# open-speech/HTK

Hardware: AMD Instinct MI355X
Metric: herest_gmm_frame_state_loglik_per_sec (higher is better)
Workload: dtype f32 (scores: bf16x3 split operands, fp32 accumulate) + f64 (alpha / beta with fp32-transcendental log-add, accumulators); 1 GPU; HERest EM iteration (pass + accumulator all-reduce + model update), 5000 tied states x 16 mix, D=39, 1250 x 500-frame utterances per GPU (BASELINE config[2]: 10k utterances sharded 8-way); states=5000, mix=16, utts_per_gpu=1250, frames=500, chunks=1, update=HERest -m 3 -v 0.01, on the device

## Files before the change

### htk_amd/csrc/fb.hip

```cpp
#include <hip/hip_runtime.h>
#include <cstdio>
#include <cstdlib>
#include <cstring>
#include <cmath>
#include <algorithm>
#include <vector>
#include <thread>
#include <mutex>
#include <condition_variable>
#include <functional>
#include "internal.h"
#include "hipcheck.h"
#include "kernels.h"
#include "devbuf.h"

static constexpr char fbOwner[] = "fb";
typedef DevBufT<fbOwner> DevBuf;

struct PrepPool {
   std::vector<std::thread> th;
   std::mutex mu;
   std::condition_variable cvGo, cvDone;
   std::function<void(int)> job;
   int generation = 0, pending = 0, nJobs = 0;
// ... 117 lines not shown
   int nUtt = 0;
   int debug = 0;
   int forceGeneral = 0;
   int noStatePath = 0;
   int noLrPath = 0;
   int topoVersion = 0;
   std::vector<unsigned char> uttFlags;
   UttClasses cls;
   size_t gamTotal = 0, betaWTotal = 0, alphaWTotal = 0;
   int totalFrames = 0, nCellsMax = 1, QMax = 1, TMax = 1, blockDim = 64;
   long long frameStates = 0;
   const float *dX = nullptr;
   DevBuf d_arena;
   DevBuf d_qLo, d_qHi, d_aLo, d_aHi, d_outp, d_beta, d_gam, d_alpha, d_pr;
   DevBuf d_betaW;
   DevBuf d_tmE, d_tmMaxP;
   DevBuf d_outpU;
   DevBuf d_alphaW, d_qBeam, d_aBeam, d_trPart, d_hits, d_hitCtl;
   DevBuf d_sink;
   DevBuf d_stCnt, d_stBucket;
   DevBuf d_laneRec;
   bool mixStateLast = false;
   bool mixDeferred = false;
   FbArgs *faMix = nullptr;
   const int *qBeamLast = nullptr;
   DevBuf d_transOff, d_trOccOff, d_counter;
   DevBuf d_rec, d_recSorted, d_recCtl;
   int recCapForce = 0;
   PrepPool *pool = nullptr; std::vector<PrepChunk> *chunks = nullptr;
   void *h_arena = nullptr; size_t h_arenaCap = 0;
   void *h_res = nullptr; size_t h_resCap = 0;
   hipEvent_t evRes = nullptr; bool resPending = false;
   bool f16Pass = false;
   hipEvent_t ev[6] = {}, evK[2] = {}, evCopy = nullptr;
   hipStream_t resStream = nullptr;
   bool timed = false, copyPending = false, scored = false;
   int evMode = 0, evModeLast = 0;
   ResLayout res() const { return {(size_t)nUtt}; }
};

static bool compat_revisit(const htkamd_model *m) { return (m->compat & HTKAMD_COMPAT_STREAM_REVISIT) && m->NSt > 1 && m->NSt != 3 && !m->tiedMix; }

extern "C" int htkamd_fb_create(htkamd_model *m, htkamd_fb **out)
{
   if (!m || !out) { htkamd_set_error("fb_create: NULL argument"); return HTKAMD_EINVAL; }
   if (m->fullc) { htkamd_set_error("fb_create: forward-backward on FULLC models is not supported yet (its mixture statistics are diagonal)"); return HTKAMD_EMODEL; }
   if (m->maxM > 4096) { htkamd_set_error("fb_create: %d mixture components per state not supported", m->maxM); return HTKAMD_EMODEL; }
   htkamd_fb *fb = new htkamd_fb();
   fb->m = m;
   auto fail = [&](const char *what, hipError_t e) { htkamd_set_error("fb_create: %s: %s", what, hipGetErrorString(e)); htkamd_fb_destroy(fb); return HTKAMD_EHIP; };
   hipError_t e;
   for (hipEvent_t *v : {&fb->ev[0], &fb->ev[1], &fb->ev[2], &fb->ev[3], &fb->ev[4], &fb->ev[5], &fb->evK[0], &fb->evK[1]})
      if ((e = hipEventCreate(v)) != hipSuccess) return fail("hipEventCreate", e);
   if ((e = hipEventCreateWithFlags(&fb->evCopy, hipEventDisableTiming)) != hipSuccess) return fail("hipEventCreate", e);
   if ((e = hipStreamCreateWithFlags(&fb->resStream, hipStreamNonBlocking)) != hipSuccess) return fail("hipStreamCreate", e);
   int rc;
   if ((rc = fb->d_counter.reserve(64)) || (rc = fb->d_transOff.reserve(sizeof(int) * (m->nT + 1))) || (rc = fb->d_trOccOff.reserve(sizeof(int) * (m->nT + 1)))) { htkamd_fb_destroy(fb); return rc; }
   if ((e = hipMemcpy(fb->d_transOff.p, m->h_transOff, sizeof(int) * (m->nT + 1), hipMemcpyHostToDevice)) != hipSuccess ||
       (e = hipMemcpy(fb->d_trOccOff.p, m->h_trOccOff, sizeof(int) * (m->nT + 1), hipMemcpyHostToDevice)) != hipSuccess) return fail("hipMemcpy", e);
   *out = fb;
   return HTKAMD_OK;
}

extern "C" void htkamd_fb_destroy(htkamd_fb *fb)
{
   if (!fb) return;
// ... 445 lines not shown

static const int clsW[4] = {1, 2, 4, 8};

static int fb_reserve_lr(htkamd_fb *fb, const htkamd_fb_config *cfg, FbArgs &fa, bool fastLadd, hipStream_t s)
{
   const htkamd_model *m = fb->m;
   int rc;
   size_t rows = 0;
   for (int W : clsW) rows += (size_t)fb->cls.of(FB_LEFT_TO_RIGHT, W).n * htkamd_stats_lr_chunks(fb->TMax) * W;
   const size_t nfr = fb->totalFrames ? fb->totalFrames : 1;
   if ((rc = fb->d_laneRec.reserve(sizeof(LaneRec) * (fb->slotState.size() + 1))) || (rc = fb->d_sink.reserve(256))) return rc;
   fa.laneRec = (LaneRec *)fb->d_laneRec.p; fa.sink = (double *)fb->d_sink.p;
   if ((rc = fb->d_alphaW.reserve(sizeof(double) * (fb->alphaWTotal + 64))) || (rc = fb->d_qBeam.reserve(sizeof(int) * (nfr + 2))) ||
       (rc = fb->d_aBeam.reserve(sizeof(int) * (nfr + 2))) || (rc = fb->d_trPart.reserve(sizeof(double) * htkamd_stats_lr_row_doubles() * (rows + 256))) ||
       (rc = fb->d_hits.reserve(sizeof(MixHit) * (rows * htkamd_stats_lr_region_cap() + 64))) || (rc = fb->d_hitCtl.reserve(sizeof(int) * (rows + 1))))
      return rc;
   fa.alphaW = (double *)fb->d_alphaW.p; fa.qBeam = (int *)fb->d_qBeam.p; fa.aBeam = (int *)fb->d_aBeam.p; fa.trPart = (double *)fb->d_trPart.p;
   fa.hits = (MixHit *)fb->d_hits.p; fa.hitCtl = (int *)fb->d_hitCtl.p; fa.nHitRegions = (int)rows; fa.hitRegionCap = htkamd_stats_lr_region_cap();
   fa.hitSlots = (m->NSt > 1 || m->tiedMix) ? 1 : 0;
   fa.qBeamNP = fb->qBeamNP.dev;
   if (htkamd_beta_lr_is_lean(fa, fastLadd)) fa.qBeam = const_cast<int *>(fb->qBeamNP.dev);
   fb->qBeamLast = fa.qBeam;
   fb->mixStateLast = false;
   fa.fastMath = fastLadd ? 1 : 0;
   if (fb->recCapForce == 0 && !fa.hitSlots && m->maxM <= 16 && (m->D == 39 || m->D == 26 || m->D == 13) &&
       (cfg->uFlags & (HTKAMD_UPMEANS | HTKAMD_UPVARS | HTKAMD_UPMIXES))) {
      size_t cap = 64;
      while (cap < 65536 && cap * (size_t)m->S < (size_t)16 * fb->totalFrames) cap <<= 1;
      while (cap > 64 && cap * (size_t)m->S * sizeof(HitS) > ((size_t)1 << 30)) cap >>= 1;
      { const char *e = getenv("HTKAMD_ST_CAP"); if (e && atoi(e) > 0) cap = (size_t)atoi(e); }
      if ((rc = fb->d_stCnt.reserve(sizeof(int) * (3 * (size_t)m->S + 4))) || (rc = fb->d_stBucket.reserve(sizeof(HitS) * cap * (size_t)m->S))) return rc;
      fb->mixStateLast = true;
      fa.stCnt = (int *)fb->d_stCnt.p; fa.nTiedStates = m->S; fa.stBucket = (HitS *)fb->d_stBucket.p; fa.stCap = (int)cap;
      HIPCHECK(hipMemsetAsync(fa.stCnt, 0, sizeof(int) * (3 * (size_t)m->S + 4), s));
   }
   return HTKAMD_OK;
}

struct FamilyKernels { int family; int (*beta)(const FbArgs &, int, bool, hipStream_t); int (*alpha)(const FbArgs &, int, bool, hipStream_t); };
static const FamilyKernels familyKernels[] = {{FB_LANE_PER_MODEL, htkamd_launch_beta_w, htkamd_launch_alpha_w},
                                              {FB_LANE_PER_STATE, htkamd_launch_beta_s, htkamd_launch_alpha_s},
                                              {FB_LEFT_TO_RIGHT, htkamd_launch_beta_lr, htkamd_launch_alpha_lr}};

static int fb_recursions(htkamd_fb *fb, const FbArgs &fa, const LdsSizes &lds, bool fastLadd, bool noEv, hipStream_t s)
{
   int rc;
   for (int pass = 0; pass < 2; pass++) {
      FbArgs fc = fa;
      const UttClasses::Range g = fb->cls.general();
      fc.uttList = fb->uttList.dev + g.first; fc.nList = g.n;
      if (g.n > 0 && (rc = pass == 0 ? htkamd_launch_beta(fc, fb->blockDim, lds.beta, s) : htkamd_launch_alpha(fc, fb->blockDim, lds.alpha, s))) return rc;
      for (const FamilyKernels &k : familyKernels)
         for (int c = 3; c >= 0; c--) {
            const UttClasses::Range r = fb->cls.of(k.family, clsW[c]);
            fc.uttList = fb->uttList.dev + r.first; fc.nList = r.n;
            if ((rc = (pass == 0 ? k.beta : k.alpha)(fc, clsW[c], fastLadd, s))) return rc;
         }
      if (!noEv) HIPCHECK(hipEventRecord(fb->ev[2 + pass], s));
   }
   return HTKAMD_OK;
}

static int fb_stats_lr(htkamd_fb *fb, const FbArgs &fa, bool fastLadd, bool noEv, hipStream_t s)
{
   int rc;
   FbArgs fc = fa;
   size_t rowOff = 0;
   for (int c = 3; c >= 0; c--) {
      const UttClasses::Range r = fb->cls.of(FB_LEFT_TO_RIGHT, clsW[c]);
      fc.uttList = fb->uttList.dev + r.first; fc.nList = r.n;
      fc.trPart = fa.trPart ? fa.trPart + rowOff * htkamd_stats_lr_row_doubles() : nullptr;
      fc.hits = fa.hits ? fa.hits + rowOff * htkamd_stats_lr_region_cap() : nullptr; fc.hitCtl = fa.hitCtl ? fa.hitCtl + rowOff : nullptr;
      rowOff += (size_t)fc.nList * htkamd_stats_lr_chunks(fb->TMax) * clsW[c];
      if ((rc = htkamd_launch_stats_lr(fc, clsW[c], fastLadd, s))) return rc;
   }
   if (!noEv) HIPCHECK(hipEventRecord(fb->ev[4], s));
   return HTKAMD_OK;
}

static int fb_mix_stats(htkamd_fb *fb, const htkamd_fb_config *cfg, FbArgs &fa, bool defer, hipStream_t s)
{
   const htkamd_model *m = fb->m;
   const int nLr = fb->cls.nLr();
   int rc;
   if (!(cfg->uFlags & (HTKAMD_UPMEANS | HTKAMD_UPVARS | HTKAMD_UPMIXES))) return HTKAMD_OK;
   if ((cfg->uFlags & (HTKAMD_UPMEANS | HTKAMD_UPVARS)) && fb->recCapForce >= 0) {
      const size_t cap = fb->recCapForce > 0 ? (size_t)fb->recCapForce : std::min<size_t>((size_t)16 * fb->totalFrames + 4096, (size_t)1 << 30);
      if ((rc = fb->d_rec.reserve(sizeof(MixRec) * cap)) || (rc = fb->d_recSorted.reserve(sizeof(MixRec) * cap)) ||
          (rc = fb->d_recCtl.reserve(sizeof(int) * (3 * ((size_t)m->G + 1) + 1 + (size_t)m->G / 2048 + 2))))
         return rc;
      fa.rec = (MixRec *)fb->d_rec.p; fa.recSorted = (MixRec *)fb->d_recSorted.p; fa.recCap = (int)cap; fa.G = m->G; fa.recCtl = (int *)fb->d_recCtl.p;
   }
   if (m->tiedMix || m->NSt > 1) {
      fa.stateCompOff = m->d_stateCompOff; fa.rec = nullptr;
      if (fb->nUtt > nLr && (rc = m->tiedMix ? htkamd_launch_mixstats_tm(fa, s) : htkamd_launch_mixstats_ms(fa, s))) return rc;
      if (nLr > 0 && (rc = htkamd_launch_mixhits_streams(fa, m->tiedMix != 0, s))) return rc;
      return HTKAMD_OK;
   }
   const bool dense = fb->nUtt > nLr && fa.gamTotal > 0, listed = nLr > 0;
   if ((rc = htkamd_launch_mixstats(fa, s, dense, listed, defer))) return rc;
   if (defer && listed && !dense && htkamd_mixstate_applies(fa)) {
      if (!fb->faMix) fb->faMix = new FbArgs();
      *fb->faMix = fa;
      fb->mixDeferred = true;
   }
   return HTKAMD_OK;
}

static int fb_execute_impl(htkamd_fb *fb, const htkamd_fb_config *cfg, htkamd_accs *accs, void *stream, bool defer)
{
   if (!fb || !cfg || !accs) { htkamd_set_error("fb_execute: NULL argument"); return HTKAMD_EINVAL; }
   fb->mixDeferred = false;
   if (accs->m != fb->m) { htkamd_set_error("fb_execute: accumulators belong to a different model"); return HTKAMD_EINVAL; }
   if (fb->nUtt == 0) return HTKAMD_OK;
   const htkamd_model *m = fb->m;
   hipStream_t s = (hipStream_t)stream;
   if (fb->topoVersion != m->topoVersion) {
      htkamd_set_error("fb_execute: the model's minimum durations changed since htkamd_fb_prepare (a re-estimated transition reached or left zero): prepare the batch again");
      return HTKAMD_EINVAL;
   }
   const ScoreArgs sa = fb_score_args(fb, cfg);
   if (cfg->scoreMode & ~(HTKAMD_SCORE_MFMA | HTKAMD_SCORE_FASTLADD | HTKAMD_SCORE_BF16 | HTKAMD_SCORE_F16 | HTKAMD_SCORE_SOUTP | HTKAMD_SCORE_DIAGC)) { htkamd_set_error("fb_execute: unknown score mode %d", cfg->scoreMode); return HTKAMD_EINVAL; }
   const bool fastLadd = (cfg->scoreMode & HTKAMD_SCORE_FASTLADD) != 0;
   FbArgs fa = fb_args(fb, cfg, accs);
   const LdsSizes lds = fb_lds_sizes(fa);

   int rc;
   if (fb->copyPending) HIPCHECK(hipStreamWaitEvent(s, fb->evCopy, 0));
   const bool noEv = fb->evMode == 1;
   HIPCHECK(hipEventRecord(fb->ev[0], s));
   if (m->tiedMix) {
      fa.tmE = (float *)fb->d_tmE.p; fa.tmMaxP = (float *)fb->d_tmMaxP.p; fa.tmPoolOff = m->d_tmPoolOff; fa.tmPool = m->tmPool; fa.totalFrames = fb->totalFrames;
      fa.tmTasks = fb->tasks.dev; fa.tmNTasks = (int)fb->tasks.size(); fa.tmSlotState = sa.slotState; fa.tmOut = sa.out;
      fa.compWeight = m->d_compWeight; fa.var = m->d_var;
      if ((rc = htkamd_launch_tm_score(fa, s))) return rc;
      fb->scored = false;
   } else {
      if ((rc = htkamd_launch_score(cfg->scoreMode, m, sa, s, fb->evK[0], fb->evK[1]))) return rc;
      fb->scored = sa.nTasks > 0;
   }
   if (m->NSt > 1) {
      if ((rc = htkamd_launch_combine_streams(fa, s))) return rc;
      if (m->maxM > 1) fa.stateCompOff = m->d_msCompOff;
   } else if (m->tiedMix) fa.stateCompOff = m->d_msCompOff;
   if (!noEv) HIPCHECK(hipEventRecord(fb->ev[1], s));
   if (fb->cls.nGeneral() > 0 && lds.alpha > 160 * 1024) { htkamd_set_error("fb_execute: %zu bytes of LDS needed (max model size %zu states)", lds.alpha, (size_t)m->maxN); return HTKAMD_EMODEL; }
   if ((rc = fb->d_betaW.reserve(sizeof(double) * (fb->betaWTotal + 8 * 512)))) return rc;
   fa.betaW = (double *)fb->d_betaW.p;
   if (fb->cls.nLr() > 0 && (rc = fb_reserve_lr(fb, cfg, fa, fastLadd, s))) return rc;
   if ((rc = fb_recursions(fb, fa, lds, fastLadd, noEv, s)) || (rc = fb_stats_lr(fb, fa, fastLadd, noEv, s)) || (rc = fb_mix_stats(fb, cfg, fa, defer, s))) return rc;
   HIPCHECK(hipEventRecord(fb->ev[5], s));
   fb->timed = true; fb->evModeLast = noEv ? 1 : 0;
   return HTKAMD_OK;
}

extern "C" int htkamd_fb_execute(htkamd_fb *fb, const htkamd_fb_config *cfg, htkamd_accs *accs, void *stream)
{
   return fb_execute_impl(fb, cfg, accs, stream, false);
}

extern "C" int htkamd_fb_execute_begin(htkamd_fb *fb, const htkamd_fb_config *cfg, htkamd_accs *accs, void *stream, int *deferred)
{
   if (deferred) *deferred = 0;
   const int rc = fb_execute_impl(fb, cfg, accs, stream, true);
   if (rc == HTKAMD_OK && deferred && fb && fb->nUtt > 0) *deferred = fb->mixDeferred ? 1 : 0;
   return rc;
}

extern "C" int htkamd_fb_execute_mix(htkamd_fb *fb, int state0, int state1, void *stream)
{
   if (!fb) { htkamd_set_error("fb_execute_mix: NULL"); return HTKAMD_EINVAL; }
   if (fb->nUtt == 0 || !fb->mixDeferred) return HTKAMD_OK;
   const int rc = htkamd_launch_mixstate_range(*fb->faMix, state0, state1, (hipStream_t)stream);
   if (rc) return rc;
   HIPCHECK(hipEventRecord(fb->ev[5], (hipStream_t)stream));
   return HTKAMD_OK;
}


static int res_staging(htkamd_fb *fb, size_t bytes)
{
   if (bytes > fb->h_resCap) {
      if (fb->h_res) (void)hipHostFree(fb->h_res);
      fb->h_res = nullptr; fb->h_resCap = 0;
      HIPCHECK(hipHostMalloc(&fb->h_res, bytes + bytes / 4, hipHostMallocDefault));
      fb->h_resCap = bytes + bytes / 4;
   }
   return HTKAMD_OK;
}

extern "C" int htkamd_fb_results_begin(htkamd_fb *fb, void *stream)
{
   if (!fb) { htkamd_set_error("fb_results_begin: NULL"); return HTKAMD_EINVAL; }
   if (fb->nUtt == 0) return HTKAMD_OK;
   hipStream_t s = (hipStream_t)stream;
   const size_t bytes = fb->res().bytes();
   int rc = res_staging(fb, bytes);
   if (rc) return rc;
   if (!fb->evRes) HIPCHECK(hipEventCreateWithFlags(&fb->evRes, hipEventDisableTiming));
   HIPCHECK(hipMemcpyAsync(fb->h_res, fb->d_pr.p, bytes, hipMemcpyDeviceToHost, s));
   HIPCHECK(hipEventRecord(fb->evRes, s));
   fb->resPending = true;
   return HTKAMD_OK;
}

extern "C" int htkamd_fb_results(htkamd_fb *fb, double *pr, int *status, void *stream)
{
   if (!fb) { htkamd_set_error("fb_results: NULL"); return HTKAMD_EINVAL; }
   hipStream_t s = (hipStream_t)stream;
   if (fb->nUtt == 0) return HTKAMD_OK;
   const size_t bytes = fb->res().bytes();
   if (fb->resPending) {
      fb->resPending = false;
      HIPCHECK(hipEventSynchronize(fb->evRes));
   } else {
      int rc = res_staging(fb, bytes);
      if (rc) return rc;
      hipStream_t cs = fb->timed ? fb->resStream : s;
      if (fb->timed) HIPCHECK(hipEventSynchronize(fb->ev[5]));
      HIPCHECK(hipMemcpyAsync(fb->h_res, fb->d_pr.p, bytes, hipMemcpyDeviceToHost, cs));
      HIPCHECK(hipStreamSynchronize(cs));
   }
   if (pr) memcpy(pr, fb->h_res, sizeof(double) * (size_t)fb->nUtt);
   if (status) memcpy(status, (const char *)fb->h_res + fb->res().status(), sizeof(int) * (size_t)fb->nUtt);
   if (fb->f16Pass) {
      int flag;
      memcpy(&flag, (const char *)fb->h_res + fb->res().flag(), sizeof(int));
      if (flag) {
         htkamd_set_error("fb_results: the fp16 scoring path met %s%s%s outside its range: nothing of this pass can be used (accumulators included) -- repeat it with HTKAMD_SCORE_BF16",
                          (flag & HTKAMD_F16_EMODEL) ? "a model coefficient" : "", (flag & HTKAMD_F16_EMODEL) && (flag & HTKAMD_F16_EFEAT) ? " and " : "", (flag & HTKAMD_F16_EFEAT) ? "a feature value" : "");
         return HTKAMD_ERANGE;
      }
   }
// ... 151 lines not shown
```

### htk_amd/csrc/fb_lr_lean.inc

```

template <int W>
__global__ __launch_bounds__(64 * W) void k_beta_np(FbArgs a)
{
   constexpr int L = 64 * W, LP = L + 2 * SPAD;
   __shared__ double xz[2][LP];
   __shared__ double prSlot;
   const int gl = threadIdx.x;
   const int li = blockIdx.x;
   if (li >= a.nList) return;
   const int u = a.uttList[li];
   const UttDesc ud = a.utt[u];
   if (ud.status != HTKAMD_UTT_OK) {
      if (gl == 0) { a.status[u] = ud.status; a.pr[u] = LZERO; }
      return;
   }
   const int T = ud.T, Q = ud.Q, nS = ud.nSlots;
   const bool valid = gl < nS;
   LrRegs s;
   load_lr(s, a, ud, gl, valid);
   store_lane_rec(a, ud, gl, valid, s);
   for (int i = gl; i < LP; i += L) { xz[0][i] = LZERO; xz[1][i] = LZERO; }
   if (gl == 0) prSlot = LZERO;
   __syncthreads();
   const int q = s.q;
   const double dSelf = (double)s.aSelf;
   const double cN = s.last ? (double)s.aExit + (double)s.aEntryNext : (double)s.aNext;
   const double dEntry = (double)s.aEntry;
   cint_lr *wB = (cint_lr *)(a.qBeamNP + ud.frame0 - 1);
   const float *row = a.outp + ud.outp0 + (size_t)(valid ? gl : 0) * T;
   double *pB = a.betaW + ud.betaW0 + gl;

   int w = wB[T];
   int lo = w & 0xffff, hi = w >> 16;
   bool in = q >= lo && q <= hi;
   constexpr int BK = 8;
   const int bT = (T - 1) / BK;
   float Rc[BK], Rn[BK];
   auto load8 = [&](float *R, const int b) {
      const f4s lo4 = *(const f4s *)(row + BK * b), hi4 = *(const f4s *)(row + BK * b + 4);
#pragma unroll
      for (int k = 0; k < 4; k++) { R[k] = lo4[k]; R[4 + k] = hi4[k]; }
// ... 469 lines not shown
         for (int o = 32; o > 0; o >>= 1) v += __shfl_xor(v, o);
         rowv[k] = v;
      }
      if (lane == 0) {
#pragma unroll
         for (int k = 0; k < 11; k++) part[k] = wantTrans ? rowv[k] : 0.0;
         part[TR_ROW - 1] = wantTrans ? (double)t0m : -1.0;
      }
   }
}

__device__ __forceinline__ double dpp_from_next(const double v, const double edge)
{
   const long long b = __double_as_longlong(v), e = __double_as_longlong(edge);
   const int lo = __builtin_amdgcn_update_dpp((int)e, (int)b, 0x130, 0xf, 0xf, false);
   const int hi = __builtin_amdgcn_update_dpp((int)(e >> 32), (int)(b >> 32), 0x130, 0xf, 0xf, false);
   return __longlong_as_double(((long long)hi << 32) | (unsigned int)lo);
}
__device__ __forceinline__ double dpp_from_prev(const double v, const double edge)
{
   const long long b = __double_as_longlong(v), e = __double_as_longlong(edge);
   const int lo = __builtin_amdgcn_update_dpp((int)e, (int)b, 0x138, 0xf, 0xf, false);
   const int hi = __builtin_amdgcn_update_dpp((int)(e >> 32), (int)(b >> 32), 0x138, 0xf, 0xf, false);
   return __longlong_as_double(((long long)hi << 32) | (unsigned int)lo);
}
typedef double d2s __attribute__((ext_vector_type(2), aligned(8)));

#define LEAN2_EU 1
__global__ __launch_bounds__(64, LEAN2_EU) void k_beta_np2(FbArgs a)
{
   constexpr int L = 128;
   const int lane = threadIdx.x, g0 = 2 * lane, g1 = g0 + 1;
   const int li = blockIdx.x;
   if (li >= a.nList) return;
   const int u = a.uttList[li];
   const UttDesc ud = a.utt[u];
   if (ud.status != HTKAMD_UTT_OK) {
      if (lane == 0) { a.status[u] = ud.status; a.pr[u] = LZERO; }
      return;
   }
   const int T = ud.T, Q = ud.Q, nS = ud.nSlots;
   const bool v0 = g0 < nS, v1 = g1 < nS;
   LrRegs s0, s1;
   load_lr(s0, a, ud, g0, v0); load_lr(s1, a, ud, g1, v1);
   store_lane_rec(a, ud, g0, v0, s0); store_lane_rec(a, ud, g1, v1, s1);
   const int q0 = s0.q, q1 = s1.q;
   const double dSelf0 = (double)s0.aSelf, dSelf1 = (double)s1.aSelf;
   const double cN0 = s0.last ? (double)s0.aExit + (double)s0.aEntryNext : (double)s0.aNext;
   const double cN1 = s1.last ? (double)s1.aExit + (double)s1.aEntryNext : (double)s1.aNext;
   cint_lr *wB = (cint_lr *)(a.qBeamNP + ud.frame0 - 1);
   const float *row0 = a.outp + ud.outp0 + (size_t)(v0 ? g0 : 0) * T, *row1 = a.outp + ud.outp0 + (size_t)(v1 ? g1 : 0) * T;
   double *pB = a.betaW + ud.betaW0 + g0;

   int w = wB[T];
   int lo = w & 0xffff, hi = w >> 16;
   bool in0 = q0 >= lo && q0 <= hi, in1 = q1 >= lo && q1 <= hi;
   constexpr int BK = 8;
   const int bT = (T - 1) / BK;
   float Rc0[BK], Rc1[BK], Rn0[BK], Rn1[BK];
   auto load8 = [&](float *R, const float *row, const int b) {
      const f4s lo4 = *(const f4s *)(row + BK * b), hi4 = *(const f4s *)(row + BK * b + 4);
#pragma unroll
      for (int k = 0; k < 4; k++) { R[k] = lo4[k]; R[4 + k] = hi4[k]; }
   };
   auto pick = [](const float *R, int k) { float v = R[0];
#pragma unroll
// ... 279 lines not shown
```

### htk_amd/csrc/gmm_bf16.hip

```cpp
#include <hip/hip_runtime.h>
#include <hip/hip_ext.h>
#include "internal.h"
#include "hipcheck.h"
#include "kernels.h"

typedef float f4 __attribute__((ext_vector_type(4)));
typedef float f4u __attribute__((ext_vector_type(4), aligned(4)));
typedef __bf16 bf8 __attribute__((ext_vector_type(8)));
typedef unsigned int u4 __attribute__((ext_vector_type(4)));
typedef const __attribute__((address_space(4))) int cint;

#define EXP2(x) __builtin_amdgcn_exp2f(x)
#define LOG2(x) __builtin_amdgcn_logf(x)
#define B16_COL_TILES 2

__device__ __forceinline__ float rows_max_b(float v)
{
   auto a = __builtin_amdgcn_permlane16_swap(__float_as_uint(v), __float_as_uint(v), false, false);
   v = fmaxf(__uint_as_float(a[0]), __uint_as_float(a[1]));
   auto b = __builtin_amdgcn_permlane32_swap(__float_as_uint(v), __float_as_uint(v), false, false);
   return fmaxf(__uint_as_float(b[0]), __uint_as_float(b[1]));
}
__device__ __forceinline__ float rows_sum_b(float v)
{
// ... 431 lines not shown
               if (3 * ks + 1 < 18) lse_slice(3 * ks + 1);
               Cc = __builtin_amdgcn_mfma_f32_32x32x16_bf16(wa[ks][0], zb[ks][1], Cc, 0, 0, 0);
               Cc = __builtin_amdgcn_mfma_f32_32x32x16_bf16(wa[ks][1], zb[ks][0], Cc, 0, 0, 0);
               if (3 * ks + 2 < 18) lse_slice(3 * ks + 2);
               Cx = __builtin_amdgcn_mfma_f32_32x32x16_bf16(wa[ks][0], zb[ks][0], Cx, 0, 0, 0);
            }
            for (int sl = 3 * KS; sl < 18; sl++) lse_slice(sl);
            asm volatile("" : "+v"(resP));
            resQ = resP; oQ = oPrev; haveQ = prevAct;
#pragma unroll
            for (int b = 0; b < 4; b++) {
               const f4 ci = __builtin_bit_cast(f4, wbuf[buf][KS * 192 + kh * 4 + b]);
#pragma unroll
               for (int r = 0; r < 4; r++) yP[4 * b + r] = (Cx[4 * b + r] + Cc[4 * b + r]) + ci[r];
            }
         }
         prevAct = actJ; oPrev += oStep;
         asm volatile("s_waitcnt vmcnt(0)" ::: "memory");
         __syncthreads();
         buf ^= 1;
      }
      if (haveQ) { if (fw + fcol < tk.nFrames) *oQ = resQ; }
      if (prevAct) {
         const float res = lse_full();
         if (fw + fcol < tk.nFrames && 2 * (nPairs - 1) + kh < tk.nSlots) *oPrev = res;
      }
   }
}

int htkamd_launch_score_bf16(const htkamd_model *m, const ScoreArgs &a, hipStream_t stream, hipEvent_t evStart, hipEvent_t evStop)
{
   if (a.nTasks <= 0) return HTKAMD_OK;
   { const int rc = htkamd_model_table_current(m, HTKAMD_SCORE_BF16, stream); if (rc) return rc; }
   if (a.qCounters == a.taskCounter + 8) HIPCHECK(hipMemsetAsync(a.taskCounter, 0, 16 * sizeof(int), stream));
   else {
      HIPCHECK(hipMemsetAsync(a.taskCounter, 0, sizeof(int), stream));
      if (a.qCounters) HIPCHECK(hipMemsetAsync(a.qCounters, 0, 8 * sizeof(int), stream));
   }
   if (m->f16Wide && (size_t)m->nTiles * ((size_t)3 * m->bf16NC * 64 * 16 + 64 * 16) >= ((size_t)1 << 32)) {
      htkamd_set_error("score_bf16: a table of %d tiles is beyond the kernel's 32-bit staging offsets", m->nTiles); return HTKAMD_EMODEL;
   }
   if (m->f16Wide) {
      dim3 block(256);
#define W_LAUNCH(KS_) do { const int b_ = a.nTasks < 256 * b16w_eu(KS_) ? a.nTasks : 256 * b16w_eu(KS_); \
                           hipExtLaunchKernelGGL((k_score_bf16w<KS_>), dim3(b_), block, 0, stream, evStart, evStop, 0, a); } while (0)
      if (m->bf16Dense) {
         W_LAUNCH(5); HIPCHECK(hipGetLastError());
         return HTKAMD_OK;
      }
      switch (m->bf16NC) {
      case 3: W_LAUNCH(6); break;
      case 2: W_LAUNCH(4); break;
      case 1: W_LAUNCH(2); break;
      default: htkamd_set_error("score_bf16: no kernel for %d K-chunks", m->bf16NC); return HTKAMD_EMODEL;
      }
#undef W_LAUNCH
      HIPCHECK(hipGetLastError());
      return HTKAMD_OK;
   }
   const int parts = B16_TASK_FRAMES / (16 * B16_COL_TILES * B16_WPB);
   int blocks = a.nTasks * parts;
   if (blocks > 256 * ((B16_COL_TILES > 2 ? 8 : 12) / B16_WPB)) blocks = 256 * ((B16_COL_TILES > 2 ? 8 : 12) / B16_WPB);
   dim3 grid(blocks), block(64 * B16_WPB);
   switch (m->bf16NC) {
   case 3: hipExtLaunchKernelGGL((k_score_bf16<3>), grid, block, 0, stream, evStart, evStop, 0, a); break;
   case 2: hipExtLaunchKernelGGL((k_score_bf16<2>), grid, block, 0, stream, evStart, evStop, 0, a); break;
   case 1: hipExtLaunchKernelGGL((k_score_bf16<1>), grid, block, 0, stream, evStart, evStop, 0, a); break;
// ... 156 lines not shown
```

### htk_amd/csrc/kernels.h

```cpp
#ifndef HTKAMD_KERNELS_H
#define HTKAMD_KERNELS_H
#include <hip/hip_runtime.h>
#include <vector>
#include "internal.h"

#define SCORE_TILE_FRAMES 128
#define B16_TASK_FRAMES 128
#define SCORE_TASK_SLOTS  16
#define SCORE_TASK_SLOTS_WIDE 64
#define SCORE_TASK_SLOTS_EXACT 8

struct ScoreTask {
   int frame0;
   int nFrames;
   int slot0;
   int nSlots;
   int outSlot0;
   int ldo;
   size_t outBase;
};

struct ScoreArgs {
   const ScoreTask *tasks = nullptr;
   int nTasks = 0;
   const float *X = nullptr;
   const int *slotState = nullptr;
   float *out = nullptr;
   const int *stateCompOff = nullptr, *compGauss = nullptr;
   const float *compLogWt = nullptr, *gparam = nullptr;
   int PS = 0, D = 0;
   double minLogExp = 0.0;
   const double *laddTab = nullptr;
   int *taskCounter = nullptr;
   const float *mfmaTab = nullptr;
   const int *stateTileOff = nullptr;
   const void *bf16Tab = nullptr;
   const void *f16Tab = nullptr;
   const int *f16Ctl = nullptr;
   int *rangeFlag = nullptr;
   const float *var = nullptr;
   int NSt = 1;
   const float *streamWt = nullptr;
   const int *qStart = nullptr;
   int *qCounters = nullptr;
   const int *slotRange = nullptr;
};

static inline ScoreArgs htkamd_score_args(const htkamd_model *m)
{
   ScoreArgs a;
   a.stateCompOff = m->d_stateCompOff; a.compGauss = m->d_compGauss; a.compLogWt = m->d_compLogWt;
   a.gparam = m->d_gparam; a.PS = m->PS; a.D = m->D; a.minLogExp = m->minLogExp; a.laddTab = m->d_laddTab;
   a.mfmaTab = m->d_mfmaTab; a.stateTileOff = m->d_stateTileOff; a.bf16Tab = m->d_bf16Tab; a.var = m->d_var;
   a.NSt = m->NSt; a.streamWt = m->d_streamWt;
   return a;
}

static inline int htkamd_tile_count(int T, int nSlots, int FR, int SL) { return ((T + FR - 1) / FR) * ((nSlots + SL - 1) / SL); }
static inline void htkamd_tile_tasks(ScoreTask *tk, int frame0, int T, int slot0, int nSlots, size_t outBase, int ldo, int FR, int SL)
{
   for (int t0 = 0; t0 < T; t0 += FR)
      for (int k0 = 0; k0 < nSlots; k0 += SL, tk++) {
         tk->frame0 = frame0 + t0; tk->nFrames = (T - t0 < FR) ? T - t0 : FR;
         tk->slot0 = slot0 + k0; tk->nSlots = (nSlots - k0 < SL) ? nSlots - k0 : SL;
         tk->outSlot0 = k0; tk->ldo = ldo; tk->outBase = outBase + (size_t)t0;
      }
}
static inline void htkamd_tile_tasks(std::vector<ScoreTask> &v, int frame0, int T, int slot0, int nSlots, size_t outBase, int ldo, int FR, int SL)
{
   if (T <= 0 || nSlots <= 0) return;
   const size_t n = v.size();
   v.resize(n + (size_t)htkamd_tile_count(T, nSlots, FR, SL));
   htkamd_tile_tasks(v.data() + n, frame0, T, slot0, nSlots, outBase, ldo, FR, SL);
}

int htkamd_launch_score_exact(const htkamd_model *m, const ScoreArgs &a, hipStream_t stream, hipEvent_t evStart = nullptr, hipEvent_t evStop = nullptr, bool soutp = false, bool diagc = false);
int htkamd_launch_score_full(const htkamd_model *m, const ScoreArgs &a, hipStream_t stream, hipEvent_t evStart, hipEvent_t evStop, bool soutp, bool diagc);
int htkamd_launch_score_mfma(const htkamd_model *m, const ScoreArgs &a, hipStream_t stream, hipEvent_t evStart = nullptr, hipEvent_t evStop = nullptr);
// ... 70 lines not shown
   htkamd_accs_layout lay;
   double pruneInit, pruneInc, pruneLim, minLogExp;
   float minFrwdP;
   int uFlags;
   size_t gamTotal;
   const size_t *gamOffByUtt;
   const int *gamChunkUtt;
   MixRec *rec, *recSorted;
   int recCap, G;
   int *recCtl;
   int NSt;
   const float *outpU;
   int compatRevisit;
   const int *nextSame;
   const int *dimStream;
   float *tmE;
   float *tmMaxP;
   const int *tmPoolOff;
   int tmPool, totalFrames;
   const ScoreTask *tmTasks; int tmNTasks; const int *tmSlotState; float *tmOut;
   const float *compWeight, *var;
   int tmCombine;
   const float *streamWt;
   MixHit *hits;
   int hitSlots;
   int *hitCtl;
   int nHitRegions, hitRegionCap;
   LaneRec *laneRec;
   const int *qBeamNP;
   int stBase;
   int *stCnt; int nTiedStates; HitS *stBucket; int stCap;
   int fastMath;
   double *sink;
};

int htkamd_launch_beta(const FbArgs &a, int blockDim, size_t lds, hipStream_t s);
int htkamd_launch_alpha(const FbArgs &a, int blockDim, size_t lds, hipStream_t s);
int htkamd_launch_mixstats(const FbArgs &a, hipStream_t s, bool dense, bool listed, bool deferState = false);
bool htkamd_mixstate_applies(const FbArgs &a);
int htkamd_launch_mixstate_range(const FbArgs &a, int st0, int st1, hipStream_t s);
int htkamd_launch_combine_streams(const FbArgs &a, hipStream_t s);
int htkamd_launch_mixstats_ms(const FbArgs &a, hipStream_t s);
int htkamd_launch_tm_score(const FbArgs &a, hipStream_t s);
int htkamd_launch_mixstats_tm(const FbArgs &a, hipStream_t s);
int htkamd_launch_mixhits_streams(const FbArgs &a, bool tied, hipStream_t s);
int htkamd_tm_score_block(const htkamd_model *m, const ScoreArgs &sa, int nRows, float tmBeam, hipStream_t s);
int htkamd_launch_beta_s(const FbArgs &a, int W, bool fast, hipStream_t s);
int htkamd_launch_alpha_s(const FbArgs &a, int W, bool fast, hipStream_t s);
int htkamd_launch_beta_w(const FbArgs &a, int W, bool fast, hipStream_t s);
int htkamd_launch_beta_lr(const FbArgs &a, int W, bool fast, hipStream_t s);
bool htkamd_beta_lr_is_lean(const FbArgs &a, bool fast);
int htkamd_launch_alpha_lr(const FbArgs &a, int W, bool fast, hipStream_t s);
int htkamd_launch_stats_lr(const FbArgs &a, int W, bool fast, hipStream_t s);
int htkamd_stats_lr_chunks(int TMax);
size_t htkamd_stats_lr_row_doubles(void);
int htkamd_stats_lr_region_cap(void);
int htkamd_launch_alpha_w(const FbArgs &a, int W, bool fast, hipStream_t s);

#endif
```

### htk_amd/csrc/update.hip

```cpp
#include <hip/hip_runtime.h>
#include <cstdlib>
#include <cstring>
#include <cmath>
#include "internal.h"
#include "hipcheck.h"

struct UpdArgs {
   int D, S, C, G, nT, H, PS, maxM;
   const int *stateCompOff, *compGauss, *transN, *transOff, *trOccOff, *hmmTrans, *hmmStateOff, *hmmState;
   float *mean, *var, *gconst, *compWeight, *transP;
   float *ivar, *gparam, *compLogWt;
   const unsigned char *rawLogWt;
   const double *acc;
   htkamd_accs_layout lay;
   int minEgs, uFlags, singleProcess, rowNormalise, hasVarFloor;
   float minVar, mixWeightFloor;
   double logTpi;
   const float *varFloor;
   unsigned char *qualT, *qualS, *qualG, *anyS, *anyG;
   unsigned char *flooredG;
   int *stats;
   int *blkStats;
   float *logVar;
   int tied;
// ... 482 lines not shown
   const int idx = blockIdx.x * blockDim.x + threadIdx.x;
   if (idx >= nTiles * 16) return;
   const int t = idx >> 4, col = idx & 15;
   int lo = 0, hi = a.S - 1;
   while (lo < hi) { const int mid = (lo + hi + 1) >> 1; if (a.stateTileOff[mid] <= t) lo = mid; else hi = mid - 1; }
   const int s = lo, c0 = a.stateCompOff[s], c1 = a.stateCompOff[s + 1];
   const int c = c0 + 16 * (t - a.stateTileOff[s]) + col;
   const int NS = a.NS, D = a.D;
   float *T = a.tab + (size_t)t * (NS + 8) * 64;
   float *ciRow = T + (size_t)(NS + (col & 3)) * 64 + (col >> 2) * 16, *endRow = ciRow + 4 * 64;
   const bool live = c < c1 && (c1 - c0 == 1 || a.compLogWt[c] > (float)LMINMIX);
   if (!live) {
      for (int j = 0; j < 16; j++) { ciRow[j] = 0.0f; endRow[j] = -1.0e30f; }
      for (int st = 0; st < NS; st++) for (int kq = 0; kq < 4; kq++) T[(size_t)st * 64 + kq * 16 + col] = 0.0f;
      return;
   }
   const int g = a.compGauss[c];
   const float *mu = a.mean + (size_t)g * D, *iv = a.ivar + (size_t)g * D;
   double q = 0.0;
   for (int i = 0; i < D; i++) q += (double)mu[i] * mu[i] * iv[i];
   const double L2E = 1.4426950408889634;
   const float ci = (float)(-0.25 * q * L2E);
   const float ce = (float)(((c1 - c0 == 1 ? 0.0 : (double)a.compLogWt[c]) - 0.5 * (double)a.gconst[g] - 0.25 * q) * L2E);
   for (int j = 0; j < 16; j++) { ciRow[j] = ci; endRow[j] = ce; }
   for (int st = 0; st < NS; st++)
      for (int kq = 0; kq < 4; kq++) {
         const int dim = 2 * st + (kq >> 1);
         float v = 0.0f;
         if (dim < D) v = (kq & 1) ? (float)((double)mu[dim] * iv[dim] * L2E) : (float)(-0.5 * (double)iv[dim] * L2E);
         T[(size_t)st * 64 + kq * 16 + col] = v;
      }
}

__global__ void k_upd_export(const int *stats, int *dst, const int *blkStats, int nBlk)
{
   int c0 = 0, c1 = 0, c2 = 0;
   for (int i = threadIdx.x; i < nBlk; i += 64) { c0 += blkStats[3 * i]; c1 += blkStats[3 * i + 1]; c2 += blkStats[3 * i + 2]; }
#pragma unroll
   for (int o = 32; o > 0; o >>= 1) { c0 += __shfl_xor(c0, o); c1 += __shfl_xor(c1, o); c2 += __shfl_xor(c2, o); }
   if (threadIdx.x < 16) dst[threadIdx.x] = stats[threadIdx.x] + (threadIdx.x == 0 ? c0 : threadIdx.x == 1 ? c1 : threadIdx.x == 5 ? c2 : 0);
}

int htkamd_model_refresh_mfma_device(htkamd_model *m, void *stream)
{
   hipStream_t s = (hipStream_t)stream;
   if (!m->d_mfmaTab) return HTKAMD_OK;
   MfmaTabArgs t;
   t.D = m->D; t.NS = m->mfmaNS; t.S = m->S; t.stateCompOff = m->d_stateCompOff; t.stateTileOff = m->d_stateTileOff; t.compGauss = m->d_compGauss;
   t.mean = m->d_mean; t.ivar = m->d_ivar; t.gconst = m->d_gconst; t.compLogWt = m->d_compLogWt; t.tab = m->d_mfmaTab;
   const int n = m->nTiles * 16;
   hipLaunchKernelGGL(k_upd_mfma, dim3((n + 255) / 256), dim3(256), 0, s, t, m->nTiles);
   HIPCHECK(hipGetLastError());
   return HTKAMD_OK;
}

extern "C" int htkamd_model_update_device_begin(htkamd_model *m, htkamd_accs *accs, const htkamd_update_config *cfg, void *stream)
{
   if (!m || !accs || !cfg) { htkamd_set_error("model_update_device: NULL argument"); return HTKAMD_EINVAL; }
   if (accs->m != m) { htkamd_set_error("model_update_device: accumulators belong to a different model"); return HTKAMD_EINVAL; }
   if (cfg->uFlags & HTKAMD_UPMAP) { htkamd_set_error("model_update_device: MAP re-estimation (HTKAMD_UPMAP) is done by htkamd_model_update"); return HTKAMD_EMODEL; }
   hipStream_t s = (hipStream_t)stream;
   int rc;
   if ((rc = htkamd_model_device_tables(m))) return rc;
   const size_t nFlag = (size_t)m->nT + 2 * (size_t)m->S + 3 * (size_t)m->G;
   const bool tied = m->h_meanLeader != nullptr;
   const size_t nTiedInts = tied ? 2 * (size_t)m->G + (size_t)m->H : 0;
   const size_t nLog = tied ? 0 : (((size_t)m->G * m->D + 3) & ~(size_t)3);
   const size_t headBytes = (((nFlag + 63) & ~(size_t)63) + 16 * sizeof(int) + sizeof(float) * (size_t)m->D + sizeof(int) * nTiedInts + 255) & ~(size_t)255;
// ... 51 lines not shown
         hipLaunchKernelGGL(k_upd_trans, dim3((m->nT + B - 1) / B), dim3(B), 0, s, a);
         hipLaunchKernelGGL(k_upd_state, dim3((m->S + B - 1) / B), dim3(B), 0, s, a);
      }
   }
   if (m->tiedMix) HIPCHECK(hipMemsetAsync(a.qualG, 1, (size_t)m->G, s));
   bool fusedG = false;
   {
      const size_t nEl = (size_t)m->G * m->D;
      const size_t ldsFused = sizeof(float) * (size_t)UPD_GPB * (m->D + m->PS) + sizeof(int) * UPD_GPB;
      if (nEl >= ((size_t)1 << 31)) { htkamd_set_error("model_update_device: %zu mean / variance elements (the element kernel indexes with 32 bits)", nEl); return HTKAMD_EMODEL; }
      if (tied) {
         hipLaunchKernelGGL(k_upd_first, dim3((m->H + B - 1) / B), dim3(B), 0, s, a);
         hipLaunchKernelGGL(k_upd_gauss_elem_tied, dim3((unsigned)((nEl + 255) / 256)), dim3(256), 0, s, a);
      } else if (!m->tiedMix && ldsFused <= 60 * 1024 && (m->PS & 3) == 0 && m->D <= 64) {
         const dim3 gr((unsigned)((m->G + UPD_GPB - 1) / UPD_GPB));
         switch ((UPD_GPB * m->D + 1023) / 1024) {
         case 1: hipLaunchKernelGGL(k_upd_gauss_fused<1>, gr, dim3(256), ldsFused, s, a); break;
         case 2: hipLaunchKernelGGL(k_upd_gauss_fused<2>, gr, dim3(256), ldsFused, s, a); break;
         case 3: hipLaunchKernelGGL(k_upd_gauss_fused<3>, gr, dim3(256), ldsFused, s, a); break;
         default: hipLaunchKernelGGL(k_upd_gauss_fused<4>, gr, dim3(256), ldsFused, s, a); break;
         }
         fusedG = true;
      } else
         hipLaunchKernelGGL(k_upd_gauss_elem, dim3((unsigned)((nEl + 1023) / 1024)), dim3(256), 0, s, a);
   }
   if (!fusedG) {
      UpdArgs ag = a;
      if (sizeof(float) * (size_t)B * m->D > 48 * 1024) ag.logVar = nullptr;
      hipLaunchKernelGGL(k_upd_gconst, dim3((m->G + B - 1) / B), dim3(B), ag.logVar ? sizeof(float) * (size_t)B * m->D : 0, s, ag);
   }
   HIPCHECK(hipGetLastError());
   if ((rc = htkamd_model_params_changed(m, s, 1))) return rc;
   const size_t nTp = (size_t)m->h_transOff[m->nT];
   if (!m->h_updPin) HIPCHECK(hipHostMalloc(&m->h_updPin, sizeof(float) * (nTp + 16), hipHostMallocDefault));
   if (!m->evUpd) { hipEvent_t e; HIPCHECK(hipEventCreateWithFlags(&e, hipEventDisableTiming)); m->evUpd = (void *)e; }
   hipLaunchKernelGGL(k_upd_export, dim3(1), dim3(64), 0, s, a.stats, (int *)(m->d_transP + nTp), a.blkStats, fusedG ? (int)((m->G + UPD_GPB - 1) / UPD_GPB) : 0);
   HIPCHECK(hipMemcpyAsync(m->h_updPin, m->d_transP, sizeof(float) * (nTp + 16), hipMemcpyDeviceToHost, s));
   HIPCHECK(hipEventRecord((hipEvent_t)m->evUpd, s));
   free(scanPosHost);
   m->updPending = 1;
   return HTKAMD_OK;
}

extern "C" int htkamd_model_update_device_end(htkamd_model *m, htkamd_update_stats *stats)
{
   if (!m || !m->updPending) { htkamd_set_error("model_update_device_end: no update in flight"); return HTKAMD_EINVAL; }
   m->updPending = 0;
   HIPCHECK(hipEventSynchronize((hipEvent_t)m->evUpd));
   const size_t nTp = (size_t)m->h_transOff[m->nT];
   int hst[16];
   memcpy(m->h_transP, m->h_updPin, sizeof(float) * nTp);
   memcpy(hst, (const float *)m->h_updPin + nTp, sizeof(hst));
   htkamd_model_refresh_topology(m);
   if (stats) {
      stats->nFloorVar = hst[0]; stats->nFloorVarMix = hst[1]; stats->nSkippedHmm = hst[2];
      stats->nNoTransOut = hst[3]; stats->nNoMixUse = hst[4]; stats->nNoVarUse = hst[5]; stats->nWeightAboveOne = hst[6];
   }
   if (hst[6] > 0) { htkamd_set_error("model_update_device: %d mixture weights above 1.001 (HERest: HError 2393)", hst[6]); return HTKAMD_EMODEL; }
   return HTKAMD_OK;
}

extern "C" int htkamd_model_update_device(htkamd_model *m, htkamd_accs *accs, const htkamd_update_config *cfg, htkamd_update_stats *stats, void *stream)
{
   const int rc = htkamd_model_update_device_begin(m, accs, cfg, stream);
   return rc ? rc : htkamd_model_update_device_end(m, stats);
}
```

Baseline: 29.49 billion frame-state log-lik/s.

## Fold counter memsets into beta kernel and write results straight to mapped host memory

The per-state counter and score task-counter memsets are now done by the first left-to-right lean beta kernel, which zeroes those words itself. The next scoring call then skips its own memset when it knows the counters are already clean. The result and update-export device-to-host memcpys are replaced by small kernels that write directly into mapped, coherent pinned host buffers, and the ev[0] record is skipped when events are off. The aim is fewer API calls and stream operations per iteration. The cost is cross-call state that tracks whether the counters are clean, plus slower zero-copy PCIe stores from kernels.

```diff
diff --git a/htk_amd/csrc/fb.hip b/htk_amd/csrc/fb.hip
--- a/htk_amd/csrc/fb.hip
+++ b/htk_amd/csrc/fb.hip
@@ -173,6 +173,7 @@
    void *h_res = nullptr; size_t h_resCap = 0;
    hipEvent_t evRes = nullptr; bool resPending = false;
    bool f16Pass = false;
+   bool scoreCntClean = false;
    hipEvent_t ev[6] = {}, evK[2] = {}, evCopy = nullptr;
    hipStream_t resStream = nullptr;
    bool timed = false, copyPending = false, scored = false;
@@ -684,8 +685,10 @@
       if ((rc = fb->d_stCnt.reserve(sizeof(int) * (3 * (size_t)m->S + 4))) || (rc = fb->d_stBucket.reserve(sizeof(HitS) * cap * (size_t)m->S))) return rc;
       fb->mixStateLast = true;
       fa.stCnt = (int *)fb->d_stCnt.p; fa.nTiedStates = m->S; fa.stBucket = (HitS *)fb->d_stBucket.p; fa.stCap = (int)cap;
-      HIPCHECK(hipMemsetAsync(fa.stCnt, 0, sizeof(int) * (3 * (size_t)m->S + 4), s));
-   }
+      if (htkamd_beta_lr_is_lean(fa, fastLadd)) { fa.zeroW[0] = fa.stCnt; fa.nZeroW[0] = 3 * m->S + 4; }
+      else HIPCHECK(hipMemsetAsync(fa.stCnt, 0, sizeof(int) * (3 * (size_t)m->S + 4), s));
+   }
+   if (htkamd_beta_lr_is_lean(fa, fastLadd)) { fa.zeroW[1] = (int *)fb->d_counter.p; fa.nZeroW[1] = 16; }
    return HTKAMD_OK;
 }
 
@@ -697,8 +700,10 @@
 static int fb_recursions(htkamd_fb *fb, const FbArgs &fa, const LdsSizes &lds, bool fastLadd, bool noEv, hipStream_t s)
 {
    int rc;
+   bool zeroed = false;
    for (int pass = 0; pass < 2; pass++) {
       FbArgs fc = fa;
+      fc.zeroW[0] = fc.zeroW[1] = nullptr;
       const UttClasses::Range g = fb->cls.general();
       fc.uttList = fb->uttList.dev + g.first; fc.nList = g.n;
       if (g.n > 0 && (rc = pass == 0 ? htkamd_launch_beta(fc, fb->blockDim, lds.beta, s) : htkamd_launch_alpha(fc, fb->blockDim, lds.alpha, s))) return rc;
@@ -706,7 +711,10 @@
          for (int c = 3; c >= 0; c--) {
             const UttClasses::Range r = fb->cls.of(k.family, clsW[c]);
             fc.uttList = fb->uttList.dev + r.first; fc.nList = r.n;
+            const bool zeroHere = pass == 0 && k.family == FB_LEFT_TO_RIGHT && r.n > 0 && !zeroed && (fa.zeroW[0] || fa.zeroW[1]);
+            if (zeroHere) { fc.zeroW[0] = fa.zeroW[0]; fc.zeroW[1] = fa.zeroW[1]; }
             if ((rc = (pass == 0 ? k.beta : k.alpha)(fc, clsW[c], fastLadd, s))) return rc;
+            if (zeroHere) { zeroed = true; fc.zeroW[0] = fc.zeroW[1] = nullptr; if (fa.zeroW[1]) fb->scoreCntClean = true; }
          }
       if (!noEv) HIPCHECK(hipEventRecord(fb->ev[2 + pass], s));
    }
@@ -771,7 +779,9 @@
       htkamd_set_error("fb_execute: the model's minimum durations changed since htkamd_fb_prepare (a re-estimated transition reached or left zero): prepare the batch again");
       return HTKAMD_EINVAL;
    }
-   const ScoreArgs sa = fb_score_args(fb, cfg);
+   ScoreArgs sa = fb_score_args(fb, cfg);
+   sa.countersZero = fb->scoreCntClean && sa.taskCounter == (int *)fb->d_counter.p;
+   fb->scoreCntClean = false;
    if (cfg->scoreMode & ~(HTKAMD_SCORE_MFMA | HTKAMD_SCORE_FASTLADD | HTKAMD_SCORE_BF16 | HTKAMD_SCORE_F16 | HTKAMD_SCORE_SOUTP | HTKAMD_SCORE_DIAGC)) { htkamd_set_error("fb_execute: unknown score mode %d", cfg->scoreMode); return HTKAMD_EINVAL; }
    const bool fastLadd = (cfg->scoreMode & HTKAMD_SCORE_FASTLADD) != 0;
    FbArgs fa = fb_args(fb, cfg, accs);
@@ -780,7 +790,7 @@
    int rc;
    if (fb->copyPending) HIPCHECK(hipStreamWaitEvent(s, fb->evCopy, 0));
    const bool noEv = fb->evMode == 1;
-   HIPCHECK(hipEventRecord(fb->ev[0], s));
+   if (!noEv) HIPCHECK(hipEventRecord(fb->ev[0], s));
    if (m->tiedMix) {
       fa.tmE = (float *)fb->d_tmE.p; fa.tmMaxP = (float *)fb->d_tmMaxP.p; fa.tmPoolOff = m->d_tmPoolOff; fa.tmPool = m->tmPool; fa.totalFrames = fb->totalFrames;
       fa.tmTasks = fb->tasks.dev; fa.tmNTasks = (int)fb->tasks.size(); fa.tmSlotState = sa.slotState; fa.tmOut = sa.out;
@@ -830,12 +840,17 @@
 }
 
 
+__global__ __launch_bounds__(256) void k_fb_results_out(const int *__restrict__ src, int *__restrict__ dst, int nWords)
+{
+   for (int i = blockIdx.x * blockDim.x + threadIdx.x; i < nWords; i += gridDim.x * blockDim.x) dst[i] = src[i];
+}
+
 static int res_staging(htkamd_fb *fb, size_t bytes)
 {
    if (bytes > fb->h_resCap) {
       if (fb->h_res) (void)hipHostFree(fb->h_res);
       fb->h_res = nullptr; fb->h_resCap = 0;
-      HIPCHECK(hipHostMalloc(&fb->h_res, bytes + bytes / 4, hipHostMallocDefault));
+      HIPCHECK(hipHostMalloc(&fb->h_res, bytes + bytes / 4, hipHostMallocMapped | hipHostMallocCoherent));
       fb->h_resCap = bytes + bytes / 4;
    }
    return HTKAMD_OK;
@@ -850,7 +865,11 @@
    int rc = res_staging(fb, bytes);
    if (rc) return rc;
    if (!fb->evRes) HIPCHECK(hipEventCreateWithFlags(&fb->evRes, hipEventDisableTiming));
-   HIPCHECK(hipMemcpyAsync(fb->h_res, fb->d_pr.p, bytes, hipMemcpyDeviceToHost, s));
+   void *dRes = nullptr;
+   HIPCHECK(hipHostGetDevicePointer(&dRes, fb->h_res, 0));
+   const int nWords = (int)(bytes / sizeof(int));
+   hipLaunchKernelGGL(k_fb_results_out, dim3((nWords + 255) / 256 < 64 ? (nWords + 255) / 256 : 64), dim3(256), 0, s, (const int *)fb->d_pr.p, (int *)dRes, nWords);
+   HIPCHECK(hipGetLastError());
    HIPCHECK(hipEventRecord(fb->evRes, s));
    fb->resPending = true;
    return HTKAMD_OK;
diff --git a/htk_amd/csrc/fb_lr_lean.inc b/htk_amd/csrc/fb_lr_lean.inc
--- a/htk_amd/csrc/fb_lr_lean.inc
+++ b/htk_amd/csrc/fb_lr_lean.inc
@@ -1,3 +1,11 @@
+
+__device__ __forceinline__ void fb_zero_words(const FbArgs &a)
+{
+   const int n = gridDim.x * blockDim.x, i0 = blockIdx.x * blockDim.x + threadIdx.x;
+#pragma unroll
+   for (int k = 0; k < 2; k++)
+      if (a.zeroW[k]) for (int i = i0; i < a.nZeroW[k]; i += n) a.zeroW[k][i] = 0;
+}
 
 template <int W>
 __global__ __launch_bounds__(64 * W) void k_beta_np(FbArgs a)
@@ -7,6 +15,7 @@
    __shared__ double prSlot;
    const int gl = threadIdx.x;
    const int li = blockIdx.x;
+   fb_zero_words(a);
    if (li >= a.nList) return;
    const int u = a.uttList[li];
    const UttDesc ud = a.utt[u];
@@ -542,6 +551,7 @@
    constexpr int L = 128;
    const int lane = threadIdx.x, g0 = 2 * lane, g1 = g0 + 1;
    const int li = blockIdx.x;
+   fb_zero_words(a);
    if (li >= a.nList) return;
    const int u = a.uttList[li];
    const UttDesc ud = a.utt[u];
diff --git a/htk_amd/csrc/gmm_bf16.hip b/htk_amd/csrc/gmm_bf16.hip
--- a/htk_amd/csrc/gmm_bf16.hip
+++ b/htk_amd/csrc/gmm_bf16.hip
@@ -487,7 +487,8 @@
 {
    if (a.nTasks <= 0) return HTKAMD_OK;
    { const int rc = htkamd_model_table_current(m, HTKAMD_SCORE_BF16, stream); if (rc) return rc; }
-   if (a.qCounters == a.taskCounter + 8) HIPCHECK(hipMemsetAsync(a.taskCounter, 0, 16 * sizeof(int), stream));
+   if (a.countersZero) ;
+   else if (a.qCounters == a.taskCounter + 8) HIPCHECK(hipMemsetAsync(a.taskCounter, 0, 16 * sizeof(int), stream));
    else {
       HIPCHECK(hipMemsetAsync(a.taskCounter, 0, sizeof(int), stream));
       if (a.qCounters) HIPCHECK(hipMemsetAsync(a.qCounters, 0, 8 * sizeof(int), stream));
diff --git a/htk_amd/csrc/kernels.h b/htk_amd/csrc/kernels.h
--- a/htk_amd/csrc/kernels.h
+++ b/htk_amd/csrc/kernels.h
@@ -44,6 +44,7 @@
    const int *qStart = nullptr;
    int *qCounters = nullptr;
    const int *slotRange = nullptr;
+   bool countersZero = false;
 };
 
 static inline ScoreArgs htkamd_score_args(const htkamd_model *m)
@@ -180,6 +181,7 @@
    int *stCnt; int nTiedStates; HitS *stBucket; int stCap;
    int fastMath;
    double *sink;
+   int *zeroW[2]; int nZeroW[2];
 };
 
 int htkamd_launch_beta(const FbArgs &a, int blockDim, size_t lds, hipStream_t s);
diff --git a/htk_amd/csrc/update.hip b/htk_amd/csrc/update.hip
--- a/htk_amd/csrc/update.hip
+++ b/htk_amd/csrc/update.hip
@@ -538,8 +538,11 @@
       }
 }
 
-__global__ void k_upd_export(const int *stats, int *dst, const int *blkStats, int nBlk)
-{
+__global__ __launch_bounds__(256) void k_upd_export(const int *stats, const int *blkStats, int nBlk, const float *__restrict__ transP, float *__restrict__ pin, int nTp)
+{
+   for (int i = blockIdx.x * blockDim.x + threadIdx.x; i < nTp; i += gridDim.x * blockDim.x) pin[i] = transP[i];
+   if (blockIdx.x != 0 || threadIdx.x >= 64) return;
+   int *dst = (int *)(pin + nTp);
    int c0 = 0, c1 = 0, c2 = 0;
    for (int i = threadIdx.x; i < nBlk; i += 64) { c0 += blkStats[3 * i]; c1 += blkStats[3 * i + 1]; c2 += blkStats[3 * i + 2]; }
 #pragma unroll
@@ -657,10 +660,15 @@
    HIPCHECK(hipGetLastError());
    if ((rc = htkamd_model_params_changed(m, s, 1))) return rc;
    const size_t nTp = (size_t)m->h_transOff[m->nT];
-   if (!m->h_updPin) HIPCHECK(hipHostMalloc(&m->h_updPin, sizeof(float) * (nTp + 16), hipHostMallocDefault));
+   if (nTp >= ((size_t)1 << 30)) { htkamd_set_error("model_update_device: %zu transition values (the export kernel indexes with 32 bits)", nTp); return HTKAMD_EMODEL; }
+   if (!m->h_updPin) HIPCHECK(hipHostMalloc(&m->h_updPin, sizeof(float) * (nTp + 16), hipHostMallocMapped | hipHostMallocCoherent));
    if (!m->evUpd) { hipEvent_t e; HIPCHECK(hipEventCreateWithFlags(&e, hipEventDisableTiming)); m->evUpd = (void *)e; }
-   hipLaunchKernelGGL(k_upd_export, dim3(1), dim3(64), 0, s, a.stats, (int *)(m->d_transP + nTp), a.blkStats, fusedG ? (int)((m->G + UPD_GPB - 1) / UPD_GPB) : 0);
-   HIPCHECK(hipMemcpyAsync(m->h_updPin, m->d_transP, sizeof(float) * (nTp + 16), hipMemcpyDeviceToHost, s));
+   void *dPin = nullptr;
+   HIPCHECK(hipHostGetDevicePointer(&dPin, m->h_updPin, 0));
+   const unsigned nbX = (unsigned)((nTp + 1023) / 1024);
+   hipLaunchKernelGGL(k_upd_export, dim3(nbX < 1 ? 1 : nbX > 256 ? 256 : nbX), dim3(256), 0, s, a.stats, a.blkStats, fusedG ? (int)((m->G + UPD_GPB - 1) / UPD_GPB) : 0,
+                      m->d_transP, (float *)dPin, (int)nTp);
+   HIPCHECK(hipGetLastError());
    HIPCHECK(hipEventRecord((hipEvent_t)m->evUpd, s));
    free(scanPosHost);
    m->updPending = 1;
```

After: 29.49 billion frame-state log-lik/s, median of 2. Within noise of the previous version (-0.0%).
